# lukehollis/three-mlagents

Hardware: AMD Instinct MI355X
Metric: env_steps_per_sec (higher is better)
Workload: dtype f32; 1 GPU; gridworld, 4096 envs/GPU, full PPO iterations: n_steps=1024, MLP pi/vf 64x64 tanh, n_epochs=10, batch_size=131072/GPU (32 minibatches/epoch), lr=3e-4, gamma=0.99, gae_lambda=0.95, clip=0.2, ent=0.01, vf=0.5, max_grad_norm=0.5; envs_per_gpu=4096, n_steps=1024, batch_size=131072, n_epochs=10, hidden=64, parallelism=single GPU

## Files before the change

### three-mlagents_amd/csrc/tma_h64.hip

```cpp
#include "tma_h64_tile.h"

#include <cstdlib>

namespace tma {

#ifdef TMA_H64_TICKS
static __device__ unsigned long long g_h64_tail_ticks;
#endif


template <int KT, int NT>
__device__ __forceinline__ void bwd_weight_acc(const float *xin, int ldx, int K, const float *dz, int ldz, int N, f32x4 (&accW)[KT][NT],
                                               float (&accb)[NT], int lane) {
    (void)K, (void)N;
    const int r16 = lane & 15, g = lane >> 4;
    float bf[NT][4];
#pragma unroll
    for (int nt = 0; nt < NT; nt++) {
        const int col = nt * 16 + r16;
#pragma unroll
        for (int s = 0; s < 4; s++) bf[nt][s] = dz[(4 * s + g) * ldz + col];
        accb[nt] += (bf[nt][0] + bf[nt][1]) + (bf[nt][2] + bf[nt][3]);
    }
#pragma unroll
    for (int kt = 0; kt < KT; kt++) {
        const int krow = kt * 16 + r16;
        float a[4];
#pragma unroll
        for (int s = 0; s < 4; s++) a[s] = xin[(4 * s + g) * ldx + krow];
#pragma unroll
        for (int s = 0; s < 4; s++)
#pragma unroll
            for (int nt = 0; nt < NT; nt++) accW[kt][nt] = mfma16(a[s], bf[nt][s], accW[kt][nt]);
    }
}

template <int KT, int NT, bool PERM = false>
__device__ __forceinline__ void flush_segment(float *stage_all, int wave, int wpb, int K, int N, const f32x4 (&accW)[KT][NT], float (&accb)[NT],
                                              float *slab_w, float *slab_b, int lane) {
    const int r16 = lane & 15, g = lane >> 4;
    const int seg = K * N + N;
    float *stage = stage_all + wave * seg;
#pragma unroll
    for (int kt = 0; kt < KT; kt++)
#pragma unroll
        for (int nt = 0; nt < NT; nt++)
#pragma unroll
            for (int r = 0; r < 4; r++) {
                const int k = kt * 16 + g * 4 + r, n = PERM ? (r16 >> 2) + 4 * (r16 & 3) : nt * 16 + r16;
                if (k < K && n < N) stage[k * N + n] = accW[kt][nt][r];
            }
#pragma unroll
    for (int nt = 0; nt < NT; nt++) {
        float v = accb[nt];
        v += __shfl_xor(v, 16, 64);
        v += __shfl_xor(v, 32, 64);
        const int n = PERM ? (r16 >> 2) + 4 * (r16 & 3) : nt * 16 + r16;
        if (g == 0 && n < N) stage[K * N + n] = v;
    }
    __syncthreads();
    for (int e = threadIdx.x; e < seg; e += blockDim.x) {
        float sum = stage_all[e];
        for (int w = 1; w < wpb; w++) sum += stage_all[w * seg + e];
        if (e < K * N) slab_w[e] = sum;
        else slab_b[e - K * N] = sum;
    }
    __syncthreads();
}

template <bool IS_PI, int DT>
__device__ __forceinline__ void grad_h64_body(const float *__restrict__ params, const PLayout &L, const Rollout &rb, const Minibatch &mb,
                                              const HParams &hp, const double *__restrict__ adv_part, int n_part, float *__restrict__ slab,
                                              double *__restrict__ stat_slot, float *smem, int n_blocks_net, int block_net) {
    __shared__ float adv_ms[2];
    const int lane = threadIdx.x & 63, wave = threadIdx.x >> 6, wpb = blockDim.x >> 6;
    const int r16 = lane & 15, g = lane >> 4;
    constexpr int H = 64;
    const int D = DT > 0 ? DT : L.D, A = L.A;
    const int ldx = ((D + 3) & ~3) + 2;
    constexpr int ld = H + 2, ld3 = 34;
    const int per_wave = 16 * (ldx + 2 * ld + ld3) + 16 * 8;
    float *wimg = smem;
    float *X = smem + IMG_FLOATS + (int64_t)wave * per_wave;
    float *h1 = X + 16 * ldx, *h2 = h1 + 16 * ld, *dzA = h2, *dzB = h1, *dz3 = h2 + 16 * ld;
    int64_t *row_off = reinterpret_cast<int64_t *>(dz3 + 16 * ld3);
    float *meta = reinterpret_cast<float *>(row_off + 16);
    const float invB = 1.0f / (float)mb.count;
    const int NOUT = IS_PI ? A : 1;
    const int KS1 = (D + 3) >> 2;
    stage_copy(params + (IS_PI ? L.img_pi : L.img_vf), wimg, IMG_FLOATS);
    if (IS_PI && hp.normalize_advantage && threadIdx.x < 64) {
        double a = 0.0, bsum = 0.0;
        for (int k = threadIdx.x; k < n_part; k += 64) a += adv_part[2 * k], bsum += adv_part[2 * k + 1];
        for (int o = 32; o > 0; o >>= 1) {
            a += __shfl_down(a, o, 64);
            bsum += __shfl_down(bsum, o, 64);
        }
        if (threadIdx.x == 0) {
            const double n = (double)mb.stats_n, mean = a / n;
            double var = n > 1.0 ? (bsum - n * mean * mean) / (n - 1.0) : 0.0;
            if (var < 0.0) var = 0.0;
            adv_ms[0] = (float)mean;
            adv_ms[1] = (float)sqrt(var);
        }
    }
    __syncthreads();
    const float amean = (IS_PI && hp.normalize_advantage) ? adv_ms[0] : 0.0f;
    const float astd = (IS_PI && hp.normalize_advantage) ? adv_ms[1] : 1.0f;
    NetAcc acc;
    zero_acc(acc);
    double st_a = 0.0, st_ent = 0.0, st_kl = 0.0, st_clip = 0.0, st_n = 0.0;
    const int64_t n_tiles = (mb.count + 15) >> 4;
    constexpr int DP_CT = (DT + 3) & ~3;
    constexpr int NV = DT > 0 ? DP_CT / 4 : 1;
    int64_t pf_off = -1;
    float pf_m0 = 0.0f, pf_m1 = 0.0f, pf_m2 = 0.0f, pf_m3 = 0.0f, pf_x[NV];
    const int64_t tile_stride = (int64_t)n_blocks_net * wpb;
    int32_t pf_noff = -1;
    bool have_noff = false;
    auto fetch = [&](int64_t tl) {
        pf_off = -1, pf_m0 = pf_m1 = pf_m2 = pf_m3 = 0.0f;
        const int32_t my_noff = pf_noff;
        if (mb.offs && lane < 16) {
            const int64_t j2 = ((tl + tile_stride) << 4) + lane;
            pf_noff = mb.offs[j2 < mb.count ? j2 : 0];
        }
        if (lane < 16 && tl < n_tiles) {
            const int64_t j = (tl << 4) + lane;
            if (j < mb.count) {
                pf_off = mb.offs ? (int64_t)(have_noff ? my_noff : mb.offs[j]) : sample_offset(mb, mb.start + j, rb.T, rb.N);
                if constexpr (IS_PI) {
                    pf_m0 = rb.log_probs[pf_off];
                    pf_m1 = rb.advantages[pf_off];
                    pf_m3 = __int_as_float(static_cast<const int32_t *>(rb.actions)[pf_off]);
                } else {
                    pf_m2 = rb.returns[pf_off];
                }
            }
        }
        if constexpr (DT > 0) {
#pragma unroll
            for (int q = 0; q < NV; q++) {
                const int e = lane + 64 * q, row = e / DP_CT, c = e - row * DP_CT;
                const int64_t orow = __shfl(pf_off, row, 64);
                pf_x[q] = (orow >= 0 && c < DT) ? rb.obs[orow * DT + c] : 0.0f;
            }
        }
    };
    auto commit = [&]() {
        if (lane < 16) {
            meta[lane * 4 + 0] = pf_m0, meta[lane * 4 + 1] = pf_m1, meta[lane * 4 + 2] = pf_m2, meta[lane * 4 + 3] = pf_m3;
            row_off[lane] = pf_off;
        }
        if constexpr (DT > 0) {
#pragma unroll
            for (int q = 0; q < NV; q++) {
                const int e = lane + 64 * q, row = e / DP_CT, c = e - row * DP_CT;
                X[row * ldx + c] = pf_x[q];
            }
        }
    };
    fetch((int64_t)block_net * wpb + wave);
    have_noff = true;
    for (int64_t tile = (int64_t)block_net * wpb + wave; tile < n_tiles; tile += tile_stride) {
        commit();
        if constexpr (DT == 0) load_obs_tile(rb.obs, row_off, D, X, ldx, lane);
        fetch(tile + tile_stride);
        dense64_tanh_lds<0>(X, ldx, KS1, wimg + IMG_W1, wimg + IMG_B1, h1, ld, lane);
        dense64_tanh_lds<16>(h1, ld, 16, wimg + IMG_W2F, wimg + IMG_B2, h2, ld, lane);
        f32x4 out[1];
        out[0] = dense64_head_lds(h2, ld, wimg + IMG_W3F, wimg + IMG_B3, lane);
#pragma unroll
        for (int r = 0; r < 4; r++) {
            const int row = g * 4 + r;
            const bool valid = row_off[row] >= 0;
            if constexpr (IS_PI) {
                const bool colok = r16 < A;
                const float x = colok ? out[0][r] : -INFINITY;
                const float m = gmax16(x);
                const float e = colok ? expf(x - m) : 0.0f;
                const float s = gsum16(e);
                const float lse = m + logf(s);
                const float lp = colok ? x - lse : 0.0f;
                const float p = e / s;
                const int act = __float_as_int(meta[row * 4 + 3]);
                const float lpa = gsum16((r16 == act) ? lp : 0.0f);
                const float ent = -gsum16(p * lp);
                const float old = meta[row * 4 + 0];
                const float advn = (meta[row * 4 + 1] - amean) / (astd + 1e-8f);
                const float ratio = expf(lpa - old);
                const float pl1 = advn * ratio;
                const float rc = fminf(fmaxf(ratio, 1.0f - hp.clip_range), 1.0f + hp.clip_range);
                const float pl2 = advn * rc;
                const float g_lp = (valid && pl1 <= pl2) ? -(advn * ratio) * invB : 0.0f;
                float dl = g_lp * (((r16 == act) ? 1.0f : 0.0f) - p);
                dl += valid ? (hp.ent_coef * invB) * (p * (lp + ent)) : 0.0f;
                dz3[row * ld3 + r16] = colok ? dl : 0.0f;
                if (valid && r16 == 0) {
                    st_a += (double)(-fminf(pl1, pl2));
                    st_ent += (double)ent;
                    st_kl += (double)((ratio - 1.0f) - (lpa - old));
                    st_clip += (fabsf(ratio - 1.0f) > hp.clip_range) ? 1.0 : 0.0;
                    st_n += 1.0;
                }
            } else {
                const float diff = out[0][r] - meta[row * 4 + 2];
                dz3[row * ld3 + r16] = (valid && r16 == 0) ? (hp.vf_coef * 2.0f * invB) * diff : 0.0f;
                if (valid && r16 == 0) st_a += (double)(diff * diff);
            }
        }
        bwd_weight_acc<4, 1>(h2, ld, H, dz3, ld3, NOUT, acc.w3, acc.b3, lane);
        dense64_bwd_input_lds<4>(dz3, ld3, wimg + IMG_W3B, h2, ld, dzA, ld, lane);
        bwd_weight_acc<4, 4>(h1, ld, H, dzA, ld, H, acc.w2, acc.b2, lane);
        dense64_bwd_input_lds<16>(dzA, ld, wimg + IMG_W2B, h1, ld, dzB, ld, lane);
        bwd_weight_acc<1, 4>(X, ldx, D, dzB, ld, H, acc.w1, acc.b1, lane);
    }
    __syncthreads();
    flush_segment<1, 4>(smem, wave, wpb, D, H, acc.w1, acc.b1, slab + (IS_PI ? L.pW1t : L.vW1t), slab + (IS_PI ? L.pb1 : L.vb1), lane);
    flush_segment<4, 4>(smem, wave, wpb, H, H, acc.w2, acc.b2, slab + (IS_PI ? L.pW2t : L.vW2t), slab + (IS_PI ? L.pb2 : L.vb2), lane);
    flush_segment<4, 1>(smem, wave, wpb, H, NOUT, acc.w3, acc.b3, slab + (IS_PI ? L.pW3t : L.vW3t), slab + (IS_PI ? L.pb3 : L.vb3), lane);
    double st[5] = {st_a, st_ent, st_kl, st_clip, st_n};
#pragma unroll
    for (int q = 0; q < 5; q++)
        for (int o = 32; o > 0; o >>= 1) st[q] += __shfl_down(st[q], o, 64);
    double *red = reinterpret_cast<double *>(smem);
    if (lane == 0)
        for (int q = 0; q < 5; q++) red[wave * 5 + q] = st[q];
    __syncthreads();
    if (threadIdx.x < 5) {
        double s = 0.0;
        for (int w = 0; w < wpb; w++) s += red[w * 5 + threadIdx.x];
        const int q = IS_PI ? (threadIdx.x == 0 ? 0 : threadIdx.x + 1) : (threadIdx.x == 0 ? 1 : -1);
        if (q >= 0) stat_slot[q] += s;
    }
}



template <bool IS_PI, int KS1C, int NWV = 8>
__device__ __forceinline__ void flush_all_t(float *stage, int wave, int lane, NetAcc &acc, const PLayout &L, int D, int NOUT, float *slab) {
    constexpr int QN = (FL_HALF + NWV - 1) / NWV;
#pragma unroll
    for (int nt = 0; nt < 4; nt++) acc.b1[nt] = xg_sum(acc.b1[nt]), acc.b2[nt] = xg_sum(acc.b2[nt]);
    acc.b3[0] = xg_sum(acc.b3[0]);
    float sums[2][QN];
    int offs[2][QN];
#pragma unroll
    for (int half = 0; half < 2; half++)
#pragma unroll
        for (int q = 0; q < QN; q++) {
            const int i = wave + NWV * q, cnt = half ? FL_REGS - FL_HALF : FL_HALF;
            offs[half][q] = i < cnt ? slab_offset_t<IS_PI, KS1C>(half * FL_HALF + i, lane, L, D, NOUT) : -1;
        }
#pragma unroll
    for (int half = 0; half < 2; half++) {
        const int base = half * FL_HALF, cnt = half ? FL_REGS - FL_HALF : FL_HALF;
        if (half) __syncthreads();
#pragma unroll
        for (int i = 0; i < FL_HALF; i++)
            if (i < cnt) stage[(wave * FL_HALF + i) * 64 + lane] = acc_reg(acc, base + i);
        __syncthreads();
#pragma unroll
        for (int q = 0; q < QN; q++) {
            const int i = wave + NWV * q;
            float sum = 0.0f;
            if (i < cnt) {
                sum = stage[i * 64 + lane];
#pragma unroll
                for (int w = 1; w < NWV; w++) sum += stage[(w * FL_HALF + i) * 64 + lane];
            }
            sums[half][q] = sum;
        }
    }
#pragma unroll
    for (int half = 0; half < 2; half++)
#pragma unroll
        for (int q = 0; q < QN; q++) {
            if (offs[half][q] >= 0) slab[offs[half][q]] = sums[half][q];
        }
}


__device__ __forceinline__ void image_store_h64(float *wimg, int D, int n_out, int x, float val) {
    constexpr int H = 64;
    if (x < D * H) {
        const int k = x >> 6, n = x & 63;
        wimg[IMG_W1 + k * 64 + (n & 15) * 4 + (n >> 4)] = val;
        return;
    }
    x -= D * H;
    if (x < H) {
        wimg[IMG_B1 + x] = val;
        return;
    }
    x -= H;
    if (x < H * H) {
        const int k = x >> 6, n = x & 63;
        wimg[IMG_W2F + k * 64 + (n & 15) * 4 + (n >> 4)] = val;
        wimg[IMG_W2B + n * 64 + (k & 15) * 4 + (k >> 4)] = val;
        return;
    }
    x -= H * H;
    if (x < H) {
        wimg[IMG_B2 + x] = val;
        return;
    }
    x -= H;
    if (x < H * n_out) {
        const int k = x / n_out, a = x - k * n_out;
        wimg[IMG_W3F + k * 16 + a] = val;
        wimg[IMG_W3B + a * 64 + (k & 15) * 4 + (k >> 4)] = val;
        return;
    }
    x -= H * n_out;
    if (x < n_out) wimg[IMG_B3 + x] = val;
}

template <bool IS_PI>
__device__ __forceinline__ void fold_adam_into_image(const AdamFold &f, const PLayout &L, float *wimg, int block_net) {
    __shared__ double fold_red[4];
    __shared__ float fold_coef;
    const int tid = threadIdx.x, nthr = blockDim.x;
    const int base = IS_PI ? L.pW1t : L.vW1t, pn = (IS_PI ? L.vW1t : L.log_std) - base, n_out = IS_PI ? L.A : 1;
    const int w2_off = L.D * 64 + 64, n_other = pn - 4096;
    const bool own_w2 = tid < 256;
    const int o_base = nthr > 256 ? 256 : 0, o_thr = nthr - o_base, o_tid = tid - o_base;
    const int nr = ((tid >> 6) & 1) * 8 + (tid & 7), kr = ((tid >> 7) & 1) * 8 + ((tid >> 3) & 7);
    constexpr int NO = 9;
    float g2[4][4], m2[4][4], v2[4][4], p2[4][4], go[NO], mo[NO], vo[NO], po[NO];
    if (own_w2) {
#pragma unroll
        for (int jj = 0; jj < 4; jj++)
#pragma unroll
            for (int j = 0; j < 4; j++) {
                const int e = base + w2_off + (kr + 16 * jj) * 64 + nr + 16 * j;
                g2[jj][j] = f.grad[e], m2[jj][j] = f.m_cur[e], v2[jj][j] = f.v_cur[e], p2[jj][j] = f.p_cur[e];
            }
    }
    if (o_tid >= 0) {
#pragma unroll
        for (int i = 0; i < NO; i++) {
            const int y = o_tid + i * o_thr, x = y < w2_off ? y : y + 4096, e = base + (y < n_other ? x : 0);
            go[i] = f.grad[e], mo[i] = f.m_cur[e], vo[i] = f.v_cur[e], po[i] = f.p_cur[e];
        }
    }
    if (tid < 256) {
        double a = tid < f.n_part ? f.sq_part[tid] : 0.0;
        for (int o = 32; o > 0; o >>= 1) a += __shfl_down(a, o, 64);
        if ((tid & 63) == 0) fold_red[tid >> 6] = a;
    }
    for (int e = tid; e < 1024; e += nthr) wimg[IMG_W1 + e] = 0.0f, wimg[IMG_W3F + e] = 0.0f, wimg[IMG_W3B + e] = 0.0f;
    if (tid < 32) wimg[IMG_B3 + tid] = 0.0f;
    __syncthreads();
    if (tid == 0) {
        const double tot = ((fold_red[0] + fold_red[1]) + fold_red[2]) + fold_red[3];
        const float total_norm = (float)sqrt(tot);
        float coef = f.max_norm / (total_norm + 1e-6f);
        coef = coef > 1.0f ? 1.0f : coef;
        if (f.max_norm <= 0.0f) coef = 1.0f;
        fold_coef = coef;
        if (IS_PI && block_net == 0) f.norm_out[0] = (double)total_norm, f.norm_out[1] = (double)coef;
    }
    __syncthreads();
    const float coef = fold_coef, inv_bc2 = 1.0f / f.bc2_sqrt;
    const bool keep = block_net == 0;
    if (own_w2) {
#pragma unroll
        for (int jj = 0; jj < 4; jj++)
#pragma unroll
            for (int j = 0; j < 4; j++) {
                const float gv = (g2[jj][j] * f.scale) * coef;
                p2[jj][j] = adam_update_h64(p2[jj][j], gv, m2[jj][j], v2[jj][j], f.beta1, f.beta2, inv_bc2, f.eps, f.lr_step);
                if (keep) {
                    const int e = base + w2_off + (kr + 16 * jj) * 64 + nr + 16 * j;
                    f.p_nxt[e] = p2[jj][j], f.m_nxt[e] = m2[jj][j], f.v_nxt[e] = v2[jj][j];
                }
            }
#pragma unroll
        for (int jj = 0; jj < 4; jj++)
            *reinterpret_cast<float4 *>(wimg + IMG_W2F + (kr + 16 * jj) * 64 + nr * 4) = float4{p2[jj][0], p2[jj][1], p2[jj][2], p2[jj][3]};
#pragma unroll
        for (int j = 0; j < 4; j++)
            *reinterpret_cast<float4 *>(wimg + IMG_W2B + (nr + 16 * j) * 64 + kr * 4) = float4{p2[0][j], p2[1][j], p2[2][j], p2[3][j]};
    }
    if (o_tid >= 0) {
#pragma unroll
        for (int i = 0; i < NO; i++) {
            const int y = o_tid + i * o_thr, x = y < w2_off ? y : y + 4096;
            if (y < n_other) {
                const float gv = (go[i] * f.scale) * coef;
                const float pnew = adam_update_h64(po[i], gv, mo[i], vo[i], f.beta1, f.beta2, inv_bc2, f.eps, f.lr_step);
                image_store_h64(wimg, L.D, n_out, x, pnew);
                if (keep) f.p_nxt[base + x] = pnew, f.m_nxt[base + x] = mo[i], f.v_nxt[base + x] = vo[i];
            }
        }
    }
}

template <bool IS_PI, int DT, bool DIRECT = false, int AT = 0>
__device__ __forceinline__ void grad_h64t_body(const float *__restrict__ params, const PLayout &L, const Rollout &rb, const Minibatch &mb,
                                               const HParams &hp, const double *__restrict__ adv_part, int n_part, float *__restrict__ slab,
                                               double *__restrict__ stat_slot, float *smem, int n_blocks_net, int block_net, const AdamFold &fold,
                                               const PrepNext &next) {
#ifdef TMA_H64_TICKS
    const unsigned long long kern_t0 = __builtin_amdgcn_s_memtime();
#endif
    __shared__ float adv_ms[2];
    const int lane = threadIdx.x & 63, wave = threadIdx.x >> 6, wpb = blockDim.x >> 6;
    const int r16 = lane & 15, g = lane >> 4;
    (void)0;
    const int D = DT > 0 ? DT : L.D, A = AT > 0 ? AT : L.A;
    constexpr int KS1C = DT > 0 ? (DT + 3) / 4 : 4;
    const int KS1 = (D + 3) >> 2;
    float *wimg = smem;
    float *slotA = smem + IMG_FLOATS + wave * T_PER_WAVE, *slotB = slotA + 16 * LDT, *dz3t = slotB + 16 * LDT, *Xt = dz3t + 256;
    const float invB = 1.0f / (float)mb.count;
    const int NOUT = IS_PI ? A : 1;
    const int64_t n_tiles = (mb.count + 15) >> 4;
    const int64_t tile_stride = (int64_t)n_blocks_net * wpb;
    auto offset_of = [&](int64_t tl) -> int32_t {
        const int64_t j = (tl << 4) + r16;
        const int64_t jc = j < mb.count ? j : 0;
        return mb.offs ? mb.offs[jc] : (int32_t)sample_offset(mb, mb.start + jc, rb.T, rb.N);
    };
    int32_t nx_off = offset_of((int64_t)block_net * wpb + wave);
    int32_t pf_off = 0;
    float pf_x[KS1C], pf_m0 = 0.0f, pf_m1 = 0.0f;
    int32_t pf_act = 0;
    const int XS = (D + 3) & ~3, RS = XS + 4;
    const float *const packed = rb.packed;
    auto fetch = [&](int64_t tl) {
        pf_off = nx_off;
        nx_off = offset_of(tl + tile_stride);
        const int64_t row = pf_off;
        if (packed) {
            const float *rec = packed + row * RS;
#pragma unroll
            for (int ks = 0; ks < KS1C; ks++) {
                const int c = 4 * ks + g;
                pf_x[ks] = rec[c < XS ? c : 0];
            }
            if constexpr (IS_PI) {
                const float4 q = *reinterpret_cast<const float4 *>(rec + XS);
                pf_m0 = q.x;
                pf_m1 = q.y;
                pf_act = __float_as_int(q.z);
            } else {
                pf_m0 = rec[XS + 3];
            }
            return;
        }
#pragma unroll
        for (int ks = 0; ks < KS1C; ks++) {
            const int c = 4 * ks + g;
            pf_x[ks] = rb.obs[row * D + (c < D ? c : 0)];
        }
        if constexpr (IS_PI) {
            pf_m0 = rb.log_probs[row];
            pf_m1 = rb.advantages[row];
            pf_act = static_cast<const int32_t *>(rb.actions)[row];
        } else {
            pf_m0 = rb.returns[row];
        }
    };
    fetch((int64_t)block_net * wpb + wave);
    if (fold.grad != nullptr) fold_adam_into_image<IS_PI>(fold, L, wimg, block_net);
    else stage_copy(params + (IS_PI ? L.img_pi : L.img_vf), wimg, IMG_FLOATS);
    if (IS_PI && hp.normalize_advantage && threadIdx.x < 64) {
        double a = 0.0, bsum = 0.0;
        for (int k = threadIdx.x; k < n_part; k += 64) a += adv_part[2 * k], bsum += adv_part[2 * k + 1];
        for (int o = 32; o > 0; o >>= 1) {
            a += __shfl_down(a, o, 64);
            bsum += __shfl_down(bsum, o, 64);
        }
        if (threadIdx.x == 0) {
            const double n = (double)mb.stats_n, mean = a / n;
            double var = n > 1.0 ? (bsum - n * mean * mean) / (n - 1.0) : 0.0;
            if (var < 0.0) var = 0.0;
            adv_ms[0] = (float)mean;
            adv_ms[1] = (float)sqrt(var);
        }
    }
    __syncthreads();
    const float amean = (IS_PI && hp.normalize_advantage) ? adv_ms[0] : 0.0f;
    const float astd = (IS_PI && hp.normalize_advantage) ? adv_ms[1] : 1.0f;
    NetAcc acc;
    zero_acc(acc);
    TileStats st;
    TileTicks tk;
    if (wave >= 4)
        for (int q = 0; q < hp.debug; q++) __builtin_amdgcn_s_sleep(100);
#ifdef TMA_H64_TICKS
    const bool tick_on = block_net == 0 && wave == 0;
    tk.on = tick_on, tk.prev = __builtin_amdgcn_s_memtime();
    const unsigned long long loop_t0 = tk.prev, loop_r0 = __builtin_amdgcn_s_memrealtime();
    if (tick_on && lane == 0) g_h64_ticks[IS_PI ? 0 : 1][12] += loop_t0 - kern_t0;
#endif
    for (int64_t tile = (int64_t)block_net * wpb + wave; tile < n_tiles; tile += tile_stride) {
        H64_TICK(15);
        const bool valid = ((tile << 4) + r16) < mb.count;
        float xb[KS1C];
#pragma unroll
        for (int ks = 0; ks < KS1C; ks++) xb[ks] = (valid && 4 * ks + g < D) ? pf_x[ks] : 0.0f;
        const float m0 = pf_m0, m1 = pf_m1;
        const int act = pf_act;
        fetch(tile + tile_stride);
        h64t_tile<IS_PI, KS1C, AT>(wimg, slotA, slotB, dz3t, Xt, xb, m0, m1, act, valid, KS1, A, invB, amean, astd, hp, acc, st, tk, lane);
    }
#ifdef TMA_H64_TICKS
    const unsigned long long loop_t1 = __builtin_amdgcn_s_memtime();
    if (tick_on && lane == 0) {
        g_h64_ticks[IS_PI ? 0 : 1][10] += loop_t1 - loop_t0;
        g_h64_ticks[IS_PI ? 0 : 1][11] += __builtin_amdgcn_s_memrealtime() - loop_r0;
    }
#endif
    __syncthreads();
#ifdef TMA_H64_TICKS
    if (tick_on && lane == 0) g_h64_ticks[IS_PI ? 0 : 1][14] += __builtin_amdgcn_s_memtime() - loop_t1;
#endif
    double *red = reinterpret_cast<double *>(smem + (DIRECT ? 4 : 8) * FL_HALF * 64);
    double stv[5] = {st.a, st.ent, st.kl, (double)st.clip, (double)st.n};
#pragma unroll
    for (int q = 0; q < 5; q++)
        for (int o = 32; o > 0; o >>= 1) stv[q] += __shfl_down(stv[q], o, 64);
    if (lane == 0)
        for (int q = 0; q < 5; q++) red[wave * 5 + q] = stv[q];
    if constexpr (DIRECT) {
        flush_all_t<IS_PI, KS1C, 4>(smem, wave, lane, acc, L, D, NOUT, slab);
    } else {
        flush_all_t<IS_PI, KS1C>(smem, wave, lane, acc, L, D, NOUT, slab);
    }
#ifdef TMA_H64_TICKS
    if (tick_on && lane == 0) g_h64_ticks[IS_PI ? 0 : 1][13] += __builtin_amdgcn_s_memtime() - loop_t1;
#endif
    if (threadIdx.x < 5) {
        double s = 0.0;
        for (int w = 0; w < wpb; w++) s += red[w * 5 + threadIdx.x];
        const int q = IS_PI ? (threadIdx.x == 0 ? 0 : threadIdx.x + 1) : (threadIdx.x == 0 ? 1 : -1);
        if (q >= 0) stat_slot[q] += s;
    }
    if constexpr (!IS_PI && !DIRECT) {
        if (next.count > 0) {
            __shared__ double prep_s1[4], prep_s2[4];
            const Minibatch nm{nullptr, next.perm_seed, next.perm_epoch, next.start, next.count, next.total, nullptr, next.count, nullptr, 0};
            int nb = (int)((next.count + 1023) / 1024);
            if (nb > ADV_BLOCKS) nb = ADV_BLOCKS;
            for (int pb = block_net; pb < nb; pb += n_blocks_net) {
                adv_partial_block(next.adv, nm, next.T, next.N, nb, pb, (int)threadIdx.x, next.partials_out, next.offs_out, next.want_sums != 0, prep_s1,
                                  prep_s2);
                __syncthreads();
            }
#ifdef TMA_H64_TICKS
            if (tick_on && lane == 0) g_h64_tail_ticks += __builtin_amdgcn_s_memtime() - loop_t1;
#endif
        }
    }
}

template <int DT, int VER, int AT = 0>
__global__ __launch_bounds__(512, 2) void ppo_grad_h64_kernel(const float *__restrict__ params, PLayout L, Rollout rb, Minibatch mb, HParams hp,
                                                              const double *__restrict__ adv_part, int n_part, float *__restrict__ slabs,
                                                              double *__restrict__ stat_slots, AdamFold fold, PrepNext next) {
    extern __shared__ __attribute__((aligned(16))) float smem[];
    const int n_pairs = gridDim.x >> 1, pair = (int)blockIdx.x % n_pairs;
    const bool pi_block = (int)blockIdx.x < n_pairs;
    float *slab = slabs + (int64_t)pair * L.P;
    double *slot = stat_slots + (int64_t)pair * 8;
    if constexpr (VER == 1) {
        if (pi_block) grad_h64_body<true, DT>(params, L, rb, mb, hp, adv_part, n_part, slab, slot, smem, n_pairs, pair);
        else grad_h64_body<false, DT>(params, L, rb, mb, hp, adv_part, n_part, slab, slot, smem, n_pairs, pair);
    } else {
        if (pi_block) grad_h64t_body<true, DT, false, AT>(params, L, rb, mb, hp, adv_part, n_part, slab, slot, smem, n_pairs, pair, fold, next);
        else grad_h64t_body<false, DT>(params, L, rb, mb, hp, adv_part, n_part, slab, slot, smem, n_pairs, pair, fold, next);
    }
}

template <int DT>
__global__ __launch_bounds__(256, 1) void ppo_grad_h64_small_kernel(const float *__restrict__ params, PLayout L, Rollout rb, Minibatch mb, HParams hp,
                                                                    const double *__restrict__ adv_part, int n_part, float *__restrict__ slabs,
                                                                    double *__restrict__ stat_slots, AdamFold fold) {
    extern __shared__ __attribute__((aligned(16))) float smem[];
    const int pair = blockIdx.x >> 1, n_pairs = gridDim.x >> 1;
    float *slab = slabs + (int64_t)pair * L.P;
    double *slot = stat_slots + (int64_t)pair * 8;
    if ((blockIdx.x & 1) == 0) grad_h64t_body<true, DT, true>(params, L, rb, mb, hp, adv_part, n_part, slab, slot, smem, n_pairs, pair, fold, PrepNext{});
    else grad_h64t_body<false, DT, true>(params, L, rb, mb, hp, adv_part, n_part, slab, slot, smem, n_pairs, pair, fold, PrepNext{});
}

}

using namespace tma;

static int grad_h64_smem_bytes(const PLayout &L, int wpb, int ver) {
    const int ldx = ((L.D + 3) & ~3) + 2, ld = L.H + 2;
    const int per_wave = ver == 1 ? 16 * (ldx + 2 * ld + 34) + 16 * 8 : T_PER_WAVE;
    const int tile = (IMG_FLOATS + wpb * per_wave) * 4;
    const int flush = wpb * (L.H * L.H + L.H) * 4;
    return tile > flush ? tile : flush;
}

static int grad_h64_version() {
    static const int ver = getenv("TMA_H64_V1") ? 1 : 2;
    return ver;
}
bool tma_grad_h64_carries_prep(int64_t count) { return grad_h64_version() == 2 && ceil_div(count, 16) > H64_BLOCKS; }

int tma_launch_grad_h64(const float *params, const PLayout &L, const Rollout &R, const Minibatch &M, const HParams &hpar, const double *adv_part,
                        int n_part, float *slabs, double *slots, int *n_slabs_out, hipStream_t s, const AdamFold *foldp, const PrepNext *nextp) {
    AdamFold fold{};
    if (foldp) fold = *foldp;
    PrepNext next{};
    if (nextp) next = *nextp;
    const int ver = grad_h64_version();
    if (ver == 1 && foldp && foldp->grad) return TMA_ERR_INVALID;
    if (next.count > 0 && !tma_grad_h64_carries_prep(M.count)) return TMA_ERR_INVALID;
    static const int stagger = getenv("TMA_H64_STAGGER") ? atoi(getenv("TMA_H64_STAGGER")) : 0;
    static const bool runtime_a = getenv("TMA_H64_RUNTIME_A") != nullptr;
    HParams hps = hpar;
    hps.debug = stagger;
    const int64_t tiles = ceil_div(M.count, 16);
    if (ver == 2 && tiles <= H64_BLOCKS) {
        const int64_t blocks = ceil_div(tiles, 4);
        const int smem = (IMG_FLOATS + 4 * T_PER_WAVE) * 4;
        auto launch_small = [&](auto k) -> int {
            TMA_HIP(hipFuncSetAttribute(reinterpret_cast<const void *>(k), hipFuncAttributeMaxDynamicSharedMemorySize, smem));
            k<<<dim3((unsigned)(2 * blocks)), dim3(256), smem, s>>>(params, L, R, M, hps, adv_part, n_part, slabs, slots, fold);
            return TMA_OK;
        };
        const int rc = L.D == 4 ? launch_small(ppo_grad_h64_small_kernel<4>) : (L.D == 6 ? launch_small(ppo_grad_h64_small_kernel<6>) : launch_small(ppo_grad_h64_small_kernel<0>));
        if (rc) return rc;
        TMA_LAUNCH_CHECK();
        *n_slabs_out = (int)blocks;
        return TMA_OK;
    }
    const int wpb4 = 8, smem4 = grad_h64_smem_bytes(L, wpb4, ver);
    int64_t blocks4 = ceil_div(tiles, wpb4);
    if (blocks4 > H64_BLOCKS) blocks4 = H64_BLOCKS;
    auto launch = [&](auto k) -> int {
        if (smem4 > 64 * 1024) TMA_HIP(hipFuncSetAttribute(reinterpret_cast<const void *>(k), hipFuncAttributeMaxDynamicSharedMemorySize, smem4));
        k<<<dim3((unsigned)(2 * blocks4)), dim3(64 * wpb4), smem4, s>>>(params, L, R, M, hps, adv_part, n_part, slabs, slots, fold, next);
        return TMA_OK;
    };
    int rc;
    if (ver == 1) rc = L.D == 4 ? launch(ppo_grad_h64_kernel<4, 1>) : (L.D == 6 ? launch(ppo_grad_h64_kernel<6, 1>) : launch(ppo_grad_h64_kernel<0, 1>));
    else if (L.D == 4 && L.A == 5 && !runtime_a) rc = launch(ppo_grad_h64_kernel<4, 2, 5>);
    else rc = L.D == 4 ? launch(ppo_grad_h64_kernel<4, 2>) : (L.D == 6 ? launch(ppo_grad_h64_kernel<6, 2>) : launch(ppo_grad_h64_kernel<0, 2>));
    if (rc) return rc;
    TMA_LAUNCH_CHECK();
    *n_slabs_out = (int)blocks4;
    return TMA_OK;
}

#ifdef TMA_H64_TICKS
extern "C" int tma_debug_h64_tail_ticks(unsigned long long *out, int reset) {
    TMA_HIP(hipDeviceSynchronize());
    if (out) TMA_HIP(hipMemcpyFromSymbol(out, HIP_SYMBOL(g_h64_tail_ticks), sizeof(unsigned long long)));
    if (reset) {
        unsigned long long z = 0;
        TMA_HIP(hipMemcpyToSymbol(HIP_SYMBOL(g_h64_tail_ticks), &z, sizeof(z)));
    }
    return TMA_OK;
}
extern "C" int tma_debug_h64_ticks(unsigned long long *out32, int reset) {
    TMA_HIP(hipDeviceSynchronize());
    if (out32) TMA_HIP(hipMemcpyFromSymbol(out32, HIP_SYMBOL(g_h64_ticks), sizeof(unsigned long long) * 32));
    if (reset) {
        unsigned long long z[32] = {};
        TMA_HIP(hipMemcpyToSymbol(HIP_SYMBOL(g_h64_ticks), z, sizeof(z)));
    }
    return TMA_OK;
}
#endif
```

Baseline: 134.5 million env-steps/s.

## Restructure grad kernel prologue to overlap Adam fold loads with row fetch

Rewrites the prologue of the h64 gradient kernel. The fused Adam-into-image fold now spreads the W2 block across all waves, issues its global loads early, and issues the advantage-partial loads up front. The first tile fetch, advantage statistics and clip-norm reduction then run between those loads and their use, and one of two __syncthreads is replaced with an LDS-only barrier. The intent is to hide global-load latency and shorten the serialized prologue before the main loop. In exchange it holds more registers live across the prologue and rejects n_part above ADV_BLOCKS.

```diff
diff --git a/three-mlagents_amd/csrc/tma_h64.hip b/three-mlagents_amd/csrc/tma_h64.hip
--- a/three-mlagents_amd/csrc/tma_h64.hip
+++ b/three-mlagents_amd/csrc/tma_h64.hip
@@ -6,6 +6,17 @@
 
 #ifdef TMA_H64_TICKS
 static __device__ unsigned long long g_h64_tail_ticks;
+static __device__ unsigned long long g_h64_edge_ticks[2][16];
+#ifndef TMA_H64_TICK_PAIR
+#define TMA_H64_TICK_PAIR 0
+#endif
+struct ProTicks {
+    unsigned long long t[5];
+};
+#define H64_PRO_STAMP(pt, i) ((pt).t[i] = __builtin_amdgcn_s_memtime())
+#else
+struct ProTicks {};
+#define H64_PRO_STAMP(pt, i) do {} while (0)
 #endif
 
 
@@ -281,121 +292,128 @@
 }
 
 
-__device__ __forceinline__ void image_store_h64(float *wimg, int D, int n_out, int x, float val) {
-    constexpr int H = 64;
-    if (x < D * H) {
-        const int k = x >> 6, n = x & 63;
-        wimg[IMG_W1 + k * 64 + (n & 15) * 4 + (n >> 4)] = val;
-        return;
-    }
-    x -= D * H;
-    if (x < H) {
-        wimg[IMG_B1 + x] = val;
-        return;
-    }
-    x -= H;
-    if (x < H * H) {
-        const int k = x >> 6, n = x & 63;
-        wimg[IMG_W2F + k * 64 + (n & 15) * 4 + (n >> 4)] = val;
-        wimg[IMG_W2B + n * 64 + (k & 15) * 4 + (k >> 4)] = val;
-        return;
-    }
-    x -= H * H;
-    if (x < H) {
-        wimg[IMG_B2 + x] = val;
-        return;
-    }
-    x -= H;
-    if (x < H * n_out) {
-        const int k = x / n_out, a = x - k * n_out;
-        wimg[IMG_W3F + k * 16 + a] = val;
-        wimg[IMG_W3B + a * 64 + (k & 15) * 4 + (k >> 4)] = val;
-        return;
-    }
-    x -= H * n_out;
-    if (x < n_out) wimg[IMG_B3 + x] = val;
-}
-
-template <bool IS_PI>
-__device__ __forceinline__ void fold_adam_into_image(const AdamFold &f, const PLayout &L, float *wimg, int block_net) {
-    __shared__ double fold_red[4];
-    __shared__ float fold_coef;
-    const int tid = threadIdx.x, nthr = blockDim.x;
-    const int base = IS_PI ? L.pW1t : L.vW1t, pn = (IS_PI ? L.vW1t : L.log_std) - base, n_out = IS_PI ? L.A : 1;
-    const int w2_off = L.D * 64 + 64, n_other = pn - 4096;
-    const bool own_w2 = tid < 256;
-    const int o_base = nthr > 256 ? 256 : 0, o_thr = nthr - o_base, o_tid = tid - o_base;
-    const int nr = ((tid >> 6) & 1) * 8 + (tid & 7), kr = ((tid >> 7) & 1) * 8 + ((tid >> 3) & 7);
-    constexpr int NO = 9;
-    float g2[4][4], m2[4][4], v2[4][4], p2[4][4], go[NO], mo[NO], vo[NO], po[NO];
-    if (own_w2) {
-#pragma unroll
-        for (int jj = 0; jj < 4; jj++)
+__device__ __forceinline__ void lds_barrier() {
+    __builtin_amdgcn_fence(__ATOMIC_RELEASE, "workgroup", "local");
+    __builtin_amdgcn_s_barrier();
+    __builtin_amdgcn_fence(__ATOMIC_ACQUIRE, "workgroup", "local");
+}
+
+__device__ __forceinline__ void image_slots_h64(int D, int n_out, int y, int &s1, int &s2) {
+    const int w1e = D * 64, w3s = w1e + 128, z = y - w3s, zc = z < 0 ? 0 : z;
+    const int k1 = y >> 6, n1 = y & 63;
+    const int k3 = zc / n_out, a3 = zc - k3 * n_out;
+    const bool head = z >= 0 && z < 64 * n_out;
+    s1 = y < w1e ? IMG_W1 + k1 * 64 + (n1 & 15) * 4 + (n1 >> 4)
+                 : (z < 0 ? IMG_B1 + (y - w1e)
+                          : (head ? IMG_W3F + k3 * 16 + a3 : IMG_B3 + (z - 64 * n_out)));
+    s2 = head ? IMG_W3B + a3 * 64 + (k3 & 15) * 4 + (k3 >> 4) : -1;
+}
+static_assert(IMG_B2 == IMG_B1 + 64, "image_slots_h64 addresses b1 and b2 as one region");
+
+template <bool IS_PI, int DT, int AT, int NTHR>
+struct AdamImageFold {
+    static_assert(NTHR == 512 || NTHR == 256, "eight-wave or four-wave workgroups");
+    static constexpr int KB = NTHR == 512 ? 2 : 4;
+    static constexpr int D_MAX = DT > 0 ? DT : 16, A_MAX = IS_PI ? (AT > 0 ? AT : 16) : 1;
+    static constexpr int NO = (D_MAX * 64 + 128 + 65 * A_MAX + NTHR - 1) / NTHR;
+    float g2[KB][4], m2[KB][4], v2[KB][4], p2[KB][4], go[NO], mo[NO], vo[NO], po[NO];
+    double sq[4];
+    int base, D, n_out, w2_off, n_other, nr, kr, k0;
+
+    __device__ __forceinline__ void issue(const AdamFold &f, const PLayout &L) {
+        const int tid = threadIdx.x;
+        base = IS_PI ? L.pW1t : L.vW1t;
+        D = DT > 0 ? DT : L.D, n_out = IS_PI ? (AT > 0 ? AT : L.A) : 1;
+        w2_off = D * 64 + 64, n_other = D * 64 + 128 + 65 * n_out;
+        nr = ((tid >> 6) & 1) * 8 + (tid & 7), kr = ((tid >> 7) & 1) * 8 + ((tid >> 3) & 7), k0 = kr + 32 * (tid >> 8);
+        if (tid < 64) {
+#pragma unroll
+            for (int u = 0; u < 4; u++) sq[u] = f.sq_part[tid + 64 * u < f.n_part ? tid + 64 * u : 0];
+        }
+    }
+    __device__ __forceinline__ void issue_state(const AdamFold &f) {
+        const int tid = threadIdx.x;
+#pragma unroll
+        for (int jj = 0; jj < KB; jj++)
 #pragma unroll
             for (int j = 0; j < 4; j++) {
-                const int e = base + w2_off + (kr + 16 * jj) * 64 + nr + 16 * j;
+                const int e = base + w2_off + (k0 + 16 * jj) * 64 + nr + 16 * j;
                 g2[jj][j] = f.grad[e], m2[jj][j] = f.m_cur[e], v2[jj][j] = f.v_cur[e], p2[jj][j] = f.p_cur[e];
             }
-    }
-    if (o_tid >= 0) {
 #pragma unroll
         for (int i = 0; i < NO; i++) {
-            const int y = o_tid + i * o_thr, x = y < w2_off ? y : y + 4096, e = base + (y < n_other ? x : 0);
+            const int y = tid + i * NTHR, x = y < w2_off ? y : y + 4096, e = base + (y < n_other ? x : 0);
             go[i] = f.grad[e], mo[i] = f.m_cur[e], vo[i] = f.v_cur[e], po[i] = f.p_cur[e];
         }
     }
-    if (tid < 256) {
-        double a = tid < f.n_part ? f.sq_part[tid] : 0.0;
-        for (int o = 32; o > 0; o >>= 1) a += __shfl_down(a, o, 64);
-        if ((tid & 63) == 0) fold_red[tid >> 6] = a;
-    }
-    for (int e = tid; e < 1024; e += nthr) wimg[IMG_W1 + e] = 0.0f, wimg[IMG_W3F + e] = 0.0f, wimg[IMG_W3B + e] = 0.0f;
-    if (tid < 32) wimg[IMG_B3 + tid] = 0.0f;
-    __syncthreads();
-    if (tid == 0) {
-        const double tot = ((fold_red[0] + fold_red[1]) + fold_red[2]) + fold_red[3];
-        const float total_norm = (float)sqrt(tot);
-        float coef = f.max_norm / (total_norm + 1e-6f);
-        coef = coef > 1.0f ? 1.0f : coef;
-        if (f.max_norm <= 0.0f) coef = 1.0f;
-        fold_coef = coef;
-        if (IS_PI && block_net == 0) f.norm_out[0] = (double)total_norm, f.norm_out[1] = (double)coef;
-    }
-    __syncthreads();
-    const float coef = fold_coef, inv_bc2 = 1.0f / f.bc2_sqrt;
-    const bool keep = block_net == 0;
-    if (own_w2) {
-#pragma unroll
-        for (int jj = 0; jj < 4; jj++)
+    __device__ __forceinline__ void zero_fill(float *wimg) const {
+        const int tid = threadIdx.x;
+#pragma unroll
+        for (int i = 0; i < 1024 / NTHR; i++) {
+            const int e = tid + i * NTHR;
+            wimg[IMG_W1 + e] = 0.0f, wimg[IMG_W3F + e] = 0.0f, wimg[IMG_W3B + e] = 0.0f;
+        }
+        if (tid < 32) wimg[IMG_B3 + tid] = 0.0f;
+    }
+    __device__ __forceinline__ void clip_coef(const AdamFold &f, int block_net, float *coef_out) const {
+        if (threadIdx.x < 64) {
+            double r[4];
+#pragma unroll
+            for (int u = 0; u < 4; u++) {
+                r[u] = (int)threadIdx.x + 64 * u < f.n_part ? sq[u] : 0.0;
+                for (int o = 32; o > 0; o >>= 1) r[u] += __shfl_down(r[u], o, 64);
+            }
+            if (threadIdx.x == 0) {
+                const double tot = ((r[0] + r[1]) + r[2]) + r[3];
+                const float total_norm = (float)sqrt(tot);
+                float coef = f.max_norm / (total_norm + 1e-6f);
+                coef = coef > 1.0f ? 1.0f : coef;
+                if (f.max_norm <= 0.0f) coef = 1.0f;
+                *coef_out = coef;
+                if (IS_PI && block_net == 0) f.norm_out[0] = (double)total_norm, f.norm_out[1] = (double)coef;
+            }
+        }
+    }
+    __device__ __forceinline__ void finish(const AdamFold &f, float *wimg, int block_net, float coef, [[maybe_unused]] ProTicks &pt) {
+        const int tid = threadIdx.x;
+        const float inv_bc2 = 1.0f / f.bc2_sqrt;
+        const bool keep = block_net == 0;
+#pragma unroll
+        for (int jj = 0; jj < KB; jj++)
 #pragma unroll
             for (int j = 0; j < 4; j++) {
                 const float gv = (g2[jj][j] * f.scale) * coef;
                 p2[jj][j] = adam_update_h64(p2[jj][j], gv, m2[jj][j], v2[jj][j], f.beta1, f.beta2, inv_bc2, f.eps, f.lr_step);
                 if (keep) {
-                    const int e = base + w2_off + (kr + 16 * jj) * 64 + nr + 16 * j;
+                    const int e = base + w2_off + (k0 + 16 * jj) * 64 + nr + 16 * j;
                     f.p_nxt[e] = p2[jj][j], f.m_nxt[e] = m2[jj][j], f.v_nxt[e] = v2[jj][j];
                 }
             }
-#pragma unroll
-        for (int jj = 0; jj < 4; jj++)
-            *reinterpret_cast<float4 *>(wimg + IMG_W2F + (kr + 16 * jj) * 64 + nr * 4) = float4{p2[jj][0], p2[jj][1], p2[jj][2], p2[jj][3]};
-#pragma unroll
-        for (int j = 0; j < 4; j++)
-            *reinterpret_cast<float4 *>(wimg + IMG_W2B + (nr + 16 * j) * 64 + kr * 4) = float4{p2[0][j], p2[1][j], p2[2][j], p2[3][j]};
-    }
-    if (o_tid >= 0) {
+        H64_PRO_STAMP(pt, 1);
+#pragma unroll
+        for (int jj = 0; jj < KB; jj++)
+            *reinterpret_cast<float4 *>(wimg + IMG_W2F + (k0 + 16 * jj) * 64 + nr * 4) = float4{p2[jj][0], p2[jj][1], p2[jj][2], p2[jj][3]};
+#pragma unroll
+        for (int j = 0; j < 4; j++) {
+            float *dst = wimg + IMG_W2B + (nr + 16 * j) * 64 + kr * 4 + (k0 >> 4);
+            if constexpr (KB == 2) *reinterpret_cast<float2 *>(dst) = float2{p2[0][j], p2[1][j]};
+            else *reinterpret_cast<float4 *>(dst) = float4{p2[0][j], p2[1][j], p2[2][j], p2[3][j]};
+        }
 #pragma unroll
         for (int i = 0; i < NO; i++) {
-            const int y = o_tid + i * o_thr, x = y < w2_off ? y : y + 4096;
+            const int y = tid + i * NTHR, x = y < w2_off ? y : y + 4096;
             if (y < n_other) {
                 const float gv = (go[i] * f.scale) * coef;
                 const float pnew = adam_update_h64(po[i], gv, mo[i], vo[i], f.beta1, f.beta2, inv_bc2, f.eps, f.lr_step);
-                image_store_h64(wimg, L.D, n_out, x, pnew);
+                int s1, s2;
+                image_slots_h64(D, n_out, y, s1, s2);
+                wimg[s1] = pnew;
+                if (s2 >= 0) wimg[s2] = pnew;
                 if (keep) f.p_nxt[base + x] = pnew, f.m_nxt[base + x] = mo[i], f.v_nxt[base + x] = vo[i];
             }
         }
     }
-}
+};
 
 template <bool IS_PI, int DT, bool DIRECT = false, int AT = 0>
 __device__ __forceinline__ void grad_h64t_body(const float *__restrict__ params, const PLayout &L, const Rollout &rb, const Minibatch &mb,
@@ -423,15 +441,29 @@
         const int64_t jc = j < mb.count ? j : 0;
         return mb.offs ? mb.offs[jc] : (int32_t)sample_offset(mb, mb.start + jc, rb.T, rb.N);
     };
+    constexpr int NTHR = DIRECT ? 256 : 512;
+    const bool adv_wave = IS_PI && hp.normalize_advantage && wave == NTHR / 64 - 1;
+    constexpr int ADV_U = ADV_BLOCKS / 64;
+    double ap_a[ADV_U], ap_b[ADV_U];
+    if (adv_wave && n_part > 0) {
+#pragma unroll
+        for (int u = 0; u < ADV_U; u++) {
+            const int k = lane + 64 * u < n_part ? lane + 64 * u : 0;
+            ap_a[u] = adv_part[2 * k], ap_b[u] = adv_part[2 * k + 1];
+        }
+    }
+    const bool folded = fold.grad != nullptr;
+    AdamImageFold<IS_PI, DT, AT, NTHR> af;
+    if (folded) af.issue(fold, L);
     int32_t nx_off = offset_of((int64_t)block_net * wpb + wave);
+    const int32_t nx2_off = offset_of((int64_t)block_net * wpb + wave + tile_stride);
+    __builtin_amdgcn_sched_barrier(0);
     int32_t pf_off = 0;
     float pf_x[KS1C], pf_m0 = 0.0f, pf_m1 = 0.0f;
     int32_t pf_act = 0;
     const int XS = (D + 3) & ~3, RS = XS + 4;
     const float *const packed = rb.packed;
-    auto fetch = [&](int64_t tl) {
-        pf_off = nx_off;
-        nx_off = offset_of(tl + tile_stride);
+    auto fetch_rows = [&]() {
         const int64_t row = pf_off;
         if (packed) {
             const float *rec = packed + row * RS;
@@ -463,25 +495,58 @@
             pf_m0 = rb.returns[row];
         }
     };
-    fetch((int64_t)block_net * wpb + wave);
-    if (fold.grad != nullptr) fold_adam_into_image<IS_PI>(fold, L, wimg, block_net);
-    else stage_copy(params + (IS_PI ? L.img_pi : L.img_vf), wimg, IMG_FLOATS);
-    if (IS_PI && hp.normalize_advantage && threadIdx.x < 64) {
-        double a = 0.0, bsum = 0.0;
-        for (int k = threadIdx.x; k < n_part; k += 64) a += adv_part[2 * k], bsum += adv_part[2 * k + 1];
-        for (int o = 32; o > 0; o >>= 1) {
-            a += __shfl_down(a, o, 64);
-            bsum += __shfl_down(bsum, o, 64);
-        }
-        if (threadIdx.x == 0) {
-            const double n = (double)mb.stats_n, mean = a / n;
-            double var = n > 1.0 ? (bsum - n * mean * mean) / (n - 1.0) : 0.0;
-            if (var < 0.0) var = 0.0;
-            adv_ms[0] = (float)mean;
-            adv_ms[1] = (float)sqrt(var);
-        }
-    }
-    __syncthreads();
+    auto fetch = [&](int64_t tl) {
+        pf_off = nx_off;
+        nx_off = offset_of(tl + tile_stride);
+        fetch_rows();
+    };
+    pf_off = nx_off, nx_off = nx2_off;
+    [[maybe_unused]] ProTicks pt;
+#ifdef TMA_H64_TICKS
+    for (int i = 0; i < 5; i++) pt.t[i] = kern_t0;
+#endif
+    __shared__ float fold_coef;
+    auto adv_stats = [&]() {
+        if (adv_wave) {
+            double a = 0.0, bsum = 0.0;
+#pragma unroll
+            for (int u = 0; u < ADV_U; u++)
+                if (lane + 64 * u < n_part) a += ap_a[u], bsum += ap_b[u];
+            for (int o = 32; o > 0; o >>= 1) {
+                a += __shfl_down(a, o, 64);
+                bsum += __shfl_down(bsum, o, 64);
+            }
+            if (lane == 0) {
+                const double n = (double)mb.stats_n, mean = a / n;
+                double var = n > 1.0 ? (bsum - n * mean * mean) / (n - 1.0) : 0.0;
+                if (var < 0.0) var = 0.0;
+                adv_ms[0] = (float)mean;
+                adv_ms[1] = (float)sqrt(var);
+            }
+        }
+    };
+    if (folded) {
+        af.issue_state(fold);
+        af.zero_fill(wimg);
+        __builtin_amdgcn_sched_barrier(0);
+        fetch_rows();
+        H64_PRO_STAMP(pt, 0);
+        adv_stats();
+        af.clip_coef(fold, block_net, &fold_coef);
+    } else {
+        fetch_rows();
+        H64_PRO_STAMP(pt, 0);
+        stage_copy(params + (IS_PI ? L.img_pi : L.img_vf), wimg, IMG_FLOATS);
+        adv_stats();
+    }
+    if (folded) {
+        lds_barrier();
+        H64_PRO_STAMP(pt, 2);
+        af.finish(fold, wimg, block_net, fold_coef, pt);
+        H64_PRO_STAMP(pt, 3);
+    }
+    lds_barrier();
+    H64_PRO_STAMP(pt, 4);
     const float amean = (IS_PI && hp.normalize_advantage) ? adv_ms[0] : 0.0f;
     const float astd = (IS_PI && hp.normalize_advantage) ? adv_ms[1] : 1.0f;
     NetAcc acc;
@@ -491,10 +556,14 @@
     if (wave >= 4)
         for (int q = 0; q < hp.debug; q++) __builtin_amdgcn_s_sleep(100);
 #ifdef TMA_H64_TICKS
-    const bool tick_on = block_net == 0 && wave == 0;
+    const bool tick_on = block_net == TMA_H64_TICK_PAIR && wave == 0;
     tk.on = tick_on, tk.prev = __builtin_amdgcn_s_memtime();
     const unsigned long long loop_t0 = tk.prev, loop_r0 = __builtin_amdgcn_s_memrealtime();
-    if (tick_on && lane == 0) g_h64_ticks[IS_PI ? 0 : 1][12] += loop_t0 - kern_t0;
+    if (tick_on && lane == 0) {
+        g_h64_ticks[IS_PI ? 0 : 1][12] += loop_t0 - kern_t0;
+        for (int i = 0; i < 5; i++) g_h64_edge_ticks[IS_PI ? 0 : 1][i] += pt.t[i] - kern_t0;
+    }
+    __shared__ unsigned long long wave_end[8];
 #endif
     for (int64_t tile = (int64_t)block_net * wpb + wave; tile < n_tiles; tile += tile_stride) {
         H64_TICK(15);
@@ -514,9 +583,13 @@
         g_h64_ticks[IS_PI ? 0 : 1][11] += __builtin_amdgcn_s_memrealtime() - loop_r0;
     }
 #endif
+#ifdef TMA_H64_TICKS
+    if (lane == 0) wave_end[wave] = loop_t1;
+#endif
     __syncthreads();
 #ifdef TMA_H64_TICKS
     if (tick_on && lane == 0) g_h64_ticks[IS_PI ? 0 : 1][14] += __builtin_amdgcn_s_memtime() - loop_t1;
+    if (block_net == TMA_H64_TICK_PAIR && lane == 0) g_h64_edge_ticks[IS_PI ? 0 : 1][8 + wave] += loop_t1 - wave_end[0];
 #endif
     double *red = reinterpret_cast<double *>(smem + (DIRECT ? 4 : 8) * FL_HALF * 64);
     double stv[5] = {st.a, st.ent, st.kl, (double)st.clip, (double)st.n};
@@ -612,6 +685,7 @@
     PrepNext next{};
     if (nextp) next = *nextp;
     const int ver = grad_h64_version();
+    if (n_part > ADV_BLOCKS) return TMA_ERR_INVALID;
     if (ver == 1 && foldp && foldp->grad) return TMA_ERR_INVALID;
     if (next.count > 0 && !tma_grad_h64_carries_prep(M.count)) return TMA_ERR_INVALID;
     static const int stagger = getenv("TMA_H64_STAGGER") ? atoi(getenv("TMA_H64_STAGGER")) : 0;
@@ -664,9 +738,11 @@
 extern "C" int tma_debug_h64_ticks(unsigned long long *out32, int reset) {
     TMA_HIP(hipDeviceSynchronize());
     if (out32) TMA_HIP(hipMemcpyFromSymbol(out32, HIP_SYMBOL(g_h64_ticks), sizeof(unsigned long long) * 32));
+    if (out32) TMA_HIP(hipMemcpyFromSymbol(out32 + 32, HIP_SYMBOL(g_h64_edge_ticks), sizeof(unsigned long long) * 32));
     if (reset) {
         unsigned long long z[32] = {};
         TMA_HIP(hipMemcpyToSymbol(HIP_SYMBOL(g_h64_ticks), z, sizeof(z)));
+        TMA_HIP(hipMemcpyToSymbol(HIP_SYMBOL(g_h64_edge_ticks), z, sizeof(z)));
     }
     return TMA_OK;
 }
```

Measured after the change: 137.2 million env-steps/s (median of 6 runs). +2.0%, better.
